# seervideodiffusion/SeerVideoLDM

Measured on AMD Instinct MI355X. Metric: UNet denoising steps/sec (12-frame 256^2 latent, 50-step DDIM), higher is better.
Workload: dtype bf16; 1 GPU; Sthv2 config: CFG batch 2 x 12 frames (2 cond + 10 predicted) x 32x32 latent, full-width SeerUNet 1.08G params, 50-step DDIM, scale 7.5; global_batch=1, parallelism=single, hip_graph=True

## Files before the change

include/seer_hip.h:

```cpp
#ifndef SEER_HIP_H
#define SEER_HIP_H

#include <stdint.h>

#ifdef __cplusplus
extern "C" {
#endif

#define SEER_OK 0
#define SEER_EINVAL (-22)
#define SEER_ENOSYS (-38)
#define SEER_ELAUNCH (-5)

#define SEER_DT_BF16 0
#define SEER_DT_F16 1

int seer_abi_version(void);
const char* seer_strerror(int code);
const char* seer_build_arch(void);

#define SEER_GEMM_PLAIN 0
#define SEER_GEMM_CONV3X3 1
#define SEER_EPI_GEGLU 1u
#define SEER_EPI_OUT_F32 2u
#define SEER_EPI_SILU 4u
#define SEER_EPI_TRANS_OUT 8u
#define SEER_EPI_ROTARY 16u
#define SEER_EPI_COLSCALE 32u

#define SEER_EPI_F16 64u
#define SEER_EPI_QUICKGELU 128u

typedef struct seer_gemm_desc {
    const void* A;
    const void* A2;
    const void* W;
    const float* bias;
    const void* residual;
    const float* rowvec;
    void* C;
    int32_t M, N, K, K1;
    int32_t lda, lda2, ldr, ldc;
    int32_t rows_per_batch, rowvec_ld;
    int32_t mode;
    uint32_t epilogue;
    int32_t Hin, Win, Cin, Hout, Wout, stride, upsample;
    int32_t batch;
    int64_t strideA, strideW, strideC;
    int32_t tile;
    int32_t splits;
    void* workspace;
    int64_t workspace_bytes;
    const float* rot_table;
    int32_t rot_tokens_per_batch, rot_pos_offset, rot_head_dim, rot_dim, rot_cols;
// ... 23 lines not shown
#define SEER_TILE_G64x64_3 8
#define SEER_TILE_G64x64_4 9
#define SEER_TILE_G64x64_5 10
#define SEER_TILE_G128x64_4 11
#define SEER_TILE_G128x160_2 12
#define SEER_TILE_G64x160_3 13
#define SEER_TILE_G256x128_2 14
#define SEER_TILE_G256x64_3 15
#define SEER_TILE_G96x160_2 16
#define SEER_TILE_G96x160_3 17
#define SEER_TILE_G96x128_2 18
#define SEER_TILE_G256x256_2 21
#define SEER_TILE_WS 19
#define SEER_TILE_T256x320 22
#define SEER_TILE_AUTO_TILED 20
#define SEER_TILE_AUTO_INVARIANT 23

int seer_gemm_bf16(const seer_gemm_desc* desc , void* stream);
int64_t seer_gemm_workspace_bytes(const seer_gemm_desc* desc );
int32_t seer_gemm_colsum_rows(const seer_gemm_desc* desc );
int32_t seer_gemm_colsum_fx_layout(const seer_gemm_desc* desc , int32_t rows_per_batch, int32_t* reps);
int32_t seer_gemm_rowstat_ok(const seer_gemm_desc* desc );
int32_t seer_gemm_lnfold_ok(const seer_gemm_desc* desc );
int64_t seer_gemm_sync_bytes(const seer_gemm_desc* desc );
#define SEER_GEMM_KERNEL_NONE 0
#define SEER_GEMM_KERNEL_TILE 1
#define SEER_GEMM_KERNEL_SPLITK 2
#define SEER_GEMM_KERNEL_WS 3
#define SEER_GEMM_KERNEL_T320 4
#define SEER_GEMM_REDUCE_NONE 0
#define SEER_GEMM_REDUCE_PLAIN 1
#define SEER_GEMM_REDUCE_COLSUM 2
#define SEER_GEMM_REDUCE_COLSUM_FX64 3
#define SEER_GEMM_REDUCE_COLSUM_FX32 4
int seer_gemm_plan(const seer_gemm_desc* desc , int32_t out[5]);

typedef struct seer_attn_desc {
    const void* Q; const void* K; const void* V; void* O;
    int64_t q_bs, k_bs, v_bs, o_bs;
    int32_t q_ss, k_ss, v_ss, o_ss;
    int32_t batch, heads, head_dim;
    int32_t Sq, Sk;
    int32_t causal;
    float scale;
    int32_t window_ws, F, H, W;
    int32_t Fq;
// ... 267 lines not shown
```

seervideoldm_amd/_lib.py:

```python
from __future__ import annotations

import ctypes as C
import os
from pathlib import Path

_PKG = Path(__file__).resolve().parent
_LIB_PATH = _PKG / "lib" / "libseer_hip.so"
_lib = None

ABI_VERSION = 27

SEER_GEMM_PLAIN = 0
SEER_GEMM_CONV3X3 = 1
SEER_EPI_GEGLU = 1
SEER_EPI_OUT_F32 = 2
SEER_EPI_SILU = 4
SEER_EPI_TRANS_OUT = 8
SEER_EPI_ROTARY = 16
SEER_EPI_COLSCALE = 32
SEER_EPI_F16 = 64
SEER_EPI_QUICKGELU = 128
SEER_ENOSYS = -38
SEER_INDEX_FROM_STEP = -1
SEER_DT_BF16, SEER_DT_F16 = 0, 1
SEER_ATTN_Q_PRESCALED = 1
SEER_ATTN_F16 = 2
SEER_TILE_AUTO, SEER_TILE_128x128, SEER_TILE_64x64, SEER_TILE_128x64 = 0, 1, 2, 3
SEER_TILE_WS = 19
SEER_TILE_AUTO_INVARIANT = 23
SEER_GEMM_KERNEL_NONE, SEER_GEMM_KERNEL_TILE, SEER_GEMM_KERNEL_SPLITK, SEER_GEMM_KERNEL_WS, SEER_GEMM_KERNEL_T320 = 0, 1, 2, 3, 4
SEER_GEMM_REDUCE_NONE, SEER_GEMM_REDUCE_PLAIN, SEER_GEMM_REDUCE_COLSUM, SEER_GEMM_REDUCE_COLSUM_FX64, SEER_GEMM_REDUCE_COLSUM_FX32 = 0, 1, 2, 3, 4


class SeerHipError(RuntimeError):
    pass


class GemmDesc(C.Structure):
    _fields_ = [
        ("A", C.c_void_p), ("A2", C.c_void_p), ("W", C.c_void_p), ("bias", C.c_void_p),
        ("residual", C.c_void_p), ("rowvec", C.c_void_p), ("C", C.c_void_p),
        ("M", C.c_int32), ("N", C.c_int32), ("K", C.c_int32), ("K1", C.c_int32),
        ("lda", C.c_int32), ("lda2", C.c_int32), ("ldr", C.c_int32), ("ldc", C.c_int32),
        ("rows_per_batch", C.c_int32), ("rowvec_ld", C.c_int32),
# ... 56 lines not shown
class AttnBwdDesc(C.Structure):
    _fields_ = [
        ("fwd", AttnDesc),
        ("dO", C.c_void_p), ("dQ", C.c_void_p), ("dK", C.c_void_p), ("dV", C.c_void_p),
        ("do_bs", C.c_int64), ("dq_bs", C.c_int64), ("dk_bs", C.c_int64), ("dv_bs", C.c_int64),
        ("do_ss", C.c_int32), ("dq_ss", C.c_int32), ("dk_ss", C.c_int32), ("dv_ss", C.c_int32),
        ("delta", C.c_void_p),
    ]


_vp, _i32, _i64, _f32, _f64 = C.c_void_p, C.c_int32, C.c_int64, C.c_float, C.c_double
_u32, _u64 = C.c_uint32, C.c_uint64

SIGNATURES = {
    "seer_abi_version": ([], C.c_int),
    "seer_strerror": ([C.c_int], C.c_char_p),
    "seer_build_arch": ([], C.c_char_p),
    "seer_gemm_bf16": ([C.POINTER(GemmDesc), _vp], C.c_int),
    "seer_gemm_workspace_bytes": ([C.POINTER(GemmDesc)], C.c_int64),
    "seer_gemm_colsum_rows": ([C.POINTER(GemmDesc)], C.c_int32),
    "seer_gemm_sync_bytes": ([C.POINTER(GemmDesc)], C.c_int64),
    "seer_gemm_rowstat_ok": ([C.POINTER(GemmDesc)], C.c_int32),
    "seer_gemm_lnfold_ok": ([C.POINTER(GemmDesc)], C.c_int32),
    "seer_gemm_plan": ([C.POINTER(GemmDesc), C.POINTER(C.c_int32)], C.c_int),
    "seer_attn_fwd": ([C.POINTER(AttnDesc), _vp], C.c_int),
    "seer_attn_causal64": ([_vp, _vp, _vp, _i32, _vp, _i32, _vp, _i32, _i32, _i32, _vp], C.c_int),
    "seer_embed_tokens": ([_vp, _i32, _i32, _vp, _i32, _vp, _i32, _i32, _vp, _i32, _vp], C.c_int),
    "seer_rotary_table": ([_vp, _i32, _i32, _vp, _vp], C.c_int),
    "seer_rotary_inplace": ([_vp, _i64, _i32, _i32, _i32, _i32, _i32, _i32, _i32, _i32, _vp, _vp], C.c_int),
    "seer_groupnorm_workspace_floats": ([_i32, _i32, _i64, _i32], C.c_int64),
    "seer_groupnorm_stats": ([_vp, _i32, _vp, _i32, _i32, _i64, _i32, _vp, _vp, _i32, _vp], C.c_int),
    "seer_groupnorm_stats_from_colsums": ([_vp, _i32, _i32, _i32, _vp, _i32, _i32, _i32, _i32, _i32, _vp, _vp], C.c_int),
    "seer_groupnorm_apply": ([_vp, _i32, _vp, _i32, _i32, _i64, _i32, _vp, _f64, _f32, _vp, _vp, _i32, _vp, _i32, _vp], C.c_int),
    "seer_groupnorm_apply_from_colsums": ([_vp, _i32, _vp, _i32, _vp, _i32, _i32, _vp, _i32, _i32, _i32, _i64, _i32, _f64, _f32, _vp, _vp, _i32,
                                           _vp, _i32, _vp], C.c_int),
    "seer_groupnorm_apply_fx": ([_vp, _i32, _vp, _i32, _vp, _i32, _vp, _i32, _i32, _i64, _i32, _f64, _f32, _vp, _vp, _i32, _vp, _vp, _i32, _vp],
                                 C.c_int),
    "seer_groupnorm_stats_fx": ([_vp, _i32, _i32, _i64, _vp, _i32, _vp], C.c_int),
    "seer_ff_fused_c320": ([_vp, _i32, _vp, _vp, _vp, _i32, _vp, _i32, _vp, _i32, _i64, _vp, _vp, C.c_float, _vp, _vp, _vp, _vp, _vp, _i64, _i32,
                            _vp, _i32, _vp], C.c_int),
    "seer_rowchain_c320": ([C.POINTER(RowChainDesc), _vp], C.c_int),
    "seer_rowchain_pack": ([_vp, _i32, _i32, _vp, _vp], C.c_int),
    "seer_ff_fused_pack_w1": ([_vp, _vp, _vp], C.c_int),
    "seer_ff_fused_pack_wcat": ([_vp, _vp, _vp], C.c_int),
    "seer_gemm_colsum_fx_layout": ([C.POINTER(GemmDesc), _i32, C.POINTER(C.c_int32)], C.c_int32),
    "seer_layernorm": ([_vp, _i64, _i32, _i32, _vp, _vp, _f32, _vp, _i32, _i32, _vp], C.c_int),
# ... 102 lines not shown
```

seervideoldm_amd/csrc/gemm.hip:

```cpp
#include "gemm_tiles.h"

namespace {

bool colsum_store_ok(const seer_gemm_desc& d) {
    return !(d.epilogue & (SEER_EPI_OUT_F32 | SEER_EPI_TRANS_OUT | SEER_EPI_GEGLU)) && d.ldc % 8 == 0 && d.N % 8 == 0 &&
           (reinterpret_cast<uintptr_t>(d.C) & 15) == 0 && (d.batch <= 1 || (d.strideC % 8) == 0);
}

int validate(seer_gemm_desc& d) {
    if (d.M <= 0 || d.N <= 0 || d.K <= 0) return SEER_EINVAL;
    if (d.K % BK) return SEER_EINVAL;
    if (!d.A || !d.W || !d.C) return SEER_EINVAL;
    const bool geglu = (d.epilogue & SEER_EPI_GEGLU) != 0;
    if (d.N % (geglu ? 32 : 4)) return SEER_EINVAL;
    if (d.mode == SEER_GEMM_CONV3X3) {
        if (d.Cin <= 0 || d.Cin % BK) return SEER_EINVAL;
        if (d.Hin <= 0 || d.Win <= 0 || d.Hout <= 0 || d.Wout <= 0) return SEER_EINVAL;
        if (d.upsample == 2) {
            if (d.K != 4 * d.Cin || d.stride != 1 || d.pad_after_only || d.Hout != 2 * d.Hin || d.Wout != 2 * d.Win) return SEER_EINVAL;
            if (d.M % (d.Hin * d.Win) || d.residual || d.rowvec) return SEER_EINVAL;
            if (d.epilogue & (SEER_EPI_OUT_F32 | SEER_EPI_TRANS_OUT | SEER_EPI_ROTARY | SEER_EPI_GEGLU)) return SEER_EINVAL;
            d.batch = 4;
            d.strideA = 0;
            d.strideW = (int64_t)d.N * d.K;
// ... 140 lines not shown
    if (d.mode != SEER_GEMM_PLAIN && d.mode != SEER_GEMM_CONV3X3) return 0;
    if (!seer_gemm_t320_eligible(d)) return 0;
    const bool geglu = (d.epilogue & SEER_EPI_GEGLU) != 0;
    const bool phases = d.mode == SEER_GEMM_CONV3X3 && d.upsample == 2;
    const bool can_split = !geglu && d.batch <= 1 && !phases && d.splits != 1;
    if (d.tile == SEER_TILE_T256x320) {
        if (!can_split) return 1;
        const int nk = d.K / BK;
        int s = d.splits > 1 ? d.splits : t320_best_split(d);
        if (s > nk / 4) s = nk / 4;
        if (s > 16) s = 16;
        if (s < 1) s = 1;
        const bool room = d.workspace && d.workspace_bytes >= seer_gemm_t320_workspace_bytes(d, s) && d.sync &&
                          d.sync_bytes >= seer_gemm_t320_sync_bytes(d, s);
        return (!assume_buffers && s > 1 && !room) ? 1 : s;
    }
    if (d.M % 256 || d.splits > 1) return 0;
    const double t = t320_model_us(d, 1);
    const double flops = 2.0 * d.M * d.N * (double)d.K * (phases ? 4 : d.batch > 1 ? d.batch : 1);
    const double rate = d.mode == SEER_GEMM_CONV3X3 ? 1.10e9 : geglu ? 0.78e9 : 0.85e9;
    return t < flops / rate ? 1 : 0;
}

struct tile_traits { int bm, bn; bool colsum_ok, ln_ok; };
tile_traits traits_of(int tile) {
    switch (tile) {
#define SEER_ROW(code, BM, BN, NS, WM, WN, MAY_SPLIT, UNIT) \
    case code: return {BM, BN, TileShape<BM, BN, NS, WM, WN>::colsum_ok, TileShape<BM, BN, NS, WM, WN>::ln_ok};
        SEER_GEMM_TILES(SEER_ROW)
#undef SEER_ROW
        default: return {};
    }
}

int launch_tiles(int tile, bool f16, const seer_gemm_desc& d, hipStream_t st) {
    switch (tile) {
#define SEER_ROW(code, BM, BN, NS, WM, WN, MAY_SPLIT, UNIT)                                                    \
    case code:                                                                                                 \
        static_assert(UNIT >= 0 && UNIT < SEER_GEMM_TILE_UNITS && (!MAY_SPLIT || (WM == 2 && WN == 2)), #code); \
        return seer_gemm_tiles_launch<UNIT>(tile, f16, d, st);
        SEER_GEMM_TILES(SEER_ROW)
#undef SEER_ROW
        default: return SEER_EINVAL;
    }
}

bool ln_resolve(const seer_gemm_desc& d, const tile_traits& tile) {
    const bool geglu = (d.epilogue & SEER_EPI_GEGLU) != 0;
    if (d.mode != SEER_GEMM_PLAIN || d.batch > 1 || (d.epilogue & (SEER_EPI_OUT_F32 | SEER_EPI_TRANS_OUT | SEER_EPI_SILU | SEER_EPI_QUICKGELU)))
        return false;
    if (d.ldc % 8 || d.N % (geglu ? 16 : 8) || (reinterpret_cast<uintptr_t>(d.C) & 15)) return false;
    if (d.rowstat && (geglu || d.colsum || d.colsum_fx)) return false;
    if (d.ln_rowstat && (d.A2 || !d.ln_wsum || (reinterpret_cast<uintptr_t>(d.ln_wsum) & 15))) return false;
    return tile.ln_ok;
}

split_choice invariant_split(const seer_gemm_desc& d) {
    const int nk = d.K / BK;
    const bool can_split = d.batch == 1 && !(d.epilogue & (SEER_EPI_GEGLU | SEER_EPI_TRANS_OUT | SEER_EPI_ROTARY)) && d.splits != 1 &&
                           !d.rowstat && !d.ln_rowstat;
    if (!can_split) return {1, SEER_TILE_AUTO};
    if (d.splits > 1) return {d.splits < nk ? d.splits : nk, SEER_TILE_G64x64_3};
    const bool conv = d.mode == SEER_GEMM_CONV3X3;
    if (conv && d.N % 160 == 0 && d.N >= 1024 && nk >= 88) return {4, SEER_TILE_G96x160_2};
    if (conv && d.N % 160 == 0 && d.N >= 512 && d.N < 1024 && nk >= 80) return {2, SEER_TILE_G96x160_2};
    if (!conv && d.N % 128 == 0 && d.N >= 1024 && nk >= 88) return {4, SEER_TILE_G128x128_2};
    return {1, SEER_TILE_AUTO};
// ... 53 lines not shown
    if (s320) {
        take(SEER_GEMM_KERNEL_T320, SEER_TILE_T256x320, s320);
    } else if (slices && !rows_ln) {
        take(SEER_GEMM_KERNEL_SPLITK, sc.tile, sc.splits);
        p.reduce = !d.colsum_fx ? (d.colsum ? SEER_GEMM_REDUCE_COLSUM : SEER_GEMM_REDUCE_PLAIN)
                 : splitk_fx_rows(d.M, inv) == 64 ? SEER_GEMM_REDUCE_COLSUM_FX64 : SEER_GEMM_REDUCE_COLSUM_FX32;
    } else {
        const bool ws = !sums && !rows_ln && seer_gemm_ws_eligible(d) &&
                        (requested == SEER_TILE_WS || (requested == SEER_TILE_AUTO && seer_gemm_ws_profitable(d)));
        take(ws ? SEER_GEMM_KERNEL_WS : SEER_GEMM_KERNEL_TILE, inv ? invariant_tile(d) : resolve_tile(d), 1);
        tile = traits_of(p.tile);
    }
    p.ln_ok = rows_ln && ln_resolve(d, tile);
    const bool split = p.kernel == SEER_GEMM_KERNEL_SPLITK;
    const int rows = !sums_stored ? 0 : s320 ? (d.M % 256 ? 0 : s320 > 1 ? 16 : 64)
                   : (p.kernel == SEER_GEMM_KERNEL_TILE && tile.colsum_ok) ? tile.bm : 0;
    p.colsum_rows = slices && sums_stored ? splitk_cs_rows(d.M, inv) : rows;
    p.colsum_fx_rows = slices && sums_stored ? splitk_fx_rows(d.M, inv) : rows;
    const bool fx_bad = d.colsum_fx && (d.colsum || d.colsum_fx_reps < 1 || d.colsum_fx_rows <= 0 || d.M % d.colsum_fx_rows ||
                                        !p.colsum_fx_rows || d.colsum_fx_rows % p.colsum_fx_rows);
    const bool sums_bad = sums && (split ? (d.epilogue & (SEER_EPI_OUT_F32 | SEER_EPI_TRANS_OUT | SEER_EPI_GEGLU)) != 0 : !rows);
    const bool tile_bad = !s320 && !split && (!tile.bm || (geglu && (d.mode == SEER_GEMM_CONV3X3 || (tile.bn / 32) % 2)));
    if (fx_bad || sums_bad || tile_bad || (rows_ln && !p.ln_ok)) p.status = SEER_EINVAL;
    if (inv) {
        if (split && !assume_buffers && !room) p.status = SEER_EINVAL;
        d.tile = SEER_TILE_AUTO_INVARIANT;
    }
    return p;
}

}

extern "C" int seer_gemm_plan(const seer_gemm_desc* desc, int32_t out[5]) {
    if (!desc || !out) return SEER_EINVAL;
    const gemm_plan p = plan_gemm(*desc, false);
    const bool ok = p.status == SEER_OK;
    out[0] = p.status; out[1] = ok ? p.kernel : 0; out[2] = ok ? p.tile : 0; out[3] = ok ? p.splits : 0; out[4] = ok ? p.reduce : 0;
    return SEER_OK;
}

extern "C" int64_t seer_gemm_workspace_bytes(const seer_gemm_desc* desc) {
    if (!desc) return SEER_EINVAL;
    const gemm_plan p = plan_gemm(*desc, true);
    if (p.kernel == SEER_GEMM_KERNEL_NONE) return p.status;
    const int s = p.tile_splits;
    const int64_t w320 = p.kernel == SEER_GEMM_KERNEL_T320 ? seer_gemm_t320_workspace_bytes(p.d, p.splits) : 0;
// ... 19 lines not shown
    if (!desc || rows_per_batch <= 0 || desc->M % rows_per_batch) return 0;
    seer_gemm_desc d = *desc;
    if (!d.colsum && !d.colsum_fx) d.colsum_fx = reinterpret_cast<int64_t*>(16);
    const int rows = plan_gemm(d, false).colsum_fx_rows;
    if (rows <= 0 || rows_per_batch % rows) return 0;
    const int adds = rows_per_batch / rows;
    if (reps) *reps = adds <= 24 ? 1 : adds <= 48 ? 2 : adds <= 96 ? 4 : 8;
    return rows;
}

extern "C" int32_t seer_gemm_rowstat_ok(const seer_gemm_desc* desc) {
    if (!desc) return 0;
    seer_gemm_desc d = *desc;
    if (!d.rowstat) d.rowstat = reinterpret_cast<int64_t*>(16);
    return plan_gemm(d, false).ln_ok ? 1 : 0;
}

extern "C" int32_t seer_gemm_lnfold_ok(const seer_gemm_desc* desc) {
    if (!desc || !desc->ln_rowstat) return 0;
    seer_gemm_desc d = *desc;
    d.ln_rowstat = nullptr;
    if (d.tile == SEER_TILE_AUTO && plan_gemm(d, false).kernel == SEER_GEMM_KERNEL_WS) return 0;
    return plan_gemm(*desc, false).ln_ok ? 1 : 0;
}

extern "C" int seer_gemm_bf16(const seer_gemm_desc* desc, void* stream) {
    if (!desc) return SEER_EINVAL;
    gemm_plan p = plan_gemm(*desc, false);
    if (p.status != SEER_OK) return p.status;
    p.d.splits = p.splits;
    hipStream_t st = reinterpret_cast<hipStream_t>(stream);
    const bool f16 = (p.d.epilogue & SEER_EPI_F16) != 0;
    switch (p.kernel) {
        case SEER_GEMM_KERNEL_T320: return seer_gemm_t320_launch(p.d, p.splits, st);
        case SEER_GEMM_KERNEL_SPLITK:
            if (const int rc = launch_tiles(p.tile, f16, p.d, st); rc != SEER_OK) return rc;
            return seer_gemm_reduce_launch(p.d, p.reduce, st);
        case SEER_GEMM_KERNEL_WS:
            if (const int rc = seer_gemm_ws_launch(p.d, st); rc != SEER_ENOSYS) return rc;
            [[fallthrough]];
        default:
            return launch_tiles(p.tile, f16, p.d, st);
    }
}
```

seervideoldm_amd/csrc/gemm_tile_kernel.h:

```cpp
#pragma once
#include "gemm_tiles.h"
#include <mutex>
#include <type_traits>

#ifdef SEER_GEMM_STAMPS
__device__ long long seer_pp8_stamps[64 * 8 * 16];
extern "C" long long* seer_lab_pp8_stamps() {
    long long* p = nullptr;
    (void)hipGetSymbolAddress(reinterpret_cast<void**>(&p), HIP_SYMBOL(seer_pp8_stamps));
    return p;
}
__device__ long long seer_block_span[8192 * 2];
extern "C" long long* seer_lab_block_span() {
    long long* p = nullptr;
    (void)hipGetSymbolAddress(reinterpret_cast<void**>(&p), HIP_SYMBOL(seer_block_span));
    return p;
}
#define PSPAN(which)                                                                                                   \
    do {                                                                                                               \
        if (threadIdx.x == 0 && blockIdx.z == 0 && blockIdx.x < 8192) seer_block_span[blockIdx.x * 2 + (which)] = wall_clock64(); \
    } while (0)
#define PSTAMP()                                                                                                       \
    do {                                                                                                               \
        if (blockIdx.x < 64 && blockIdx.z == 0 && (threadIdx.x & 63) == 0 && nst_ < 16)                                \
// ... 28 lines not shown

    extern __shared__ __attribute__((aligned(16))) unsigned char smem[];
    constexpr int STAGE = TS::STAGE;
    bf16* const smem_b = reinterpret_cast<bf16*>(smem);

    [[maybe_unused]] int nst_ = 0;
    const int tid = threadIdx.x;
    const int lane = tid & 63;
    const int wave = __builtin_amdgcn_readfirstlane(tid >> 6);
    const int wm = wave / WN, wn = wave % WN;
    PSTAMP();
    PSPAN(0);

    const int tiles_m = (p.M + BM - 1) / BM;
    const int tiles_n = (p.N + BN - 1) / BN;
    const int nwg = tiles_m * tiles_n;
    int wg;
    {
        const int L = blockIdx.x;
        const int xcd = L & 7;
        const int q = nwg >> 3, r = nwg & 7;
        wg = (xcd < r ? xcd * (q + 1) : r * (q + 1) + (xcd - r) * q) + (L >> 3);
    }
#ifndef SEER_GEMM_GM
#define SEER_GEMM_GM 4
#endif
    constexpr int GM = SEER_GEMM_GM;
    const int group = wg / (GM * tiles_n);
    const int first_m = group * GM;
    const int gsz = min(tiles_m - first_m, GM);
    const int tm = first_m + (wg % (GM * tiles_n)) % gsz;
    const int tn = (wg % (GM * tiles_n)) / gsz;
    const int m0 = tm * BM, n0 = tn * BN;

    const int z = SPLIT ? 0 : blockIdx.z;
    const bf16* __restrict__ A = reinterpret_cast<const bf16*>(p.A) + (int64_t)z * p.strideA;
    const bf16* __restrict__ A2 = reinterpret_cast<const bf16*>(p.A2);
    const bf16* __restrict__ W = reinterpret_cast<const bf16*>(p.W) + (int64_t)z * p.strideW;

    const int c8 = (tid & 7) * 8;
    const int srow = tid >> 3;
    int64_t a_off[A_CH];
    int64_t a_off2[A_CH];
    int a_oy[A_CH], a_ox[A_CH];
    auto a_tile_row = [&](int c) { return PP8 ? (wave >> 2) * 128 + (c >> 1) * 64 + 16 * (wave & 3) + 8 * (c & 1) + (lane >> 3) : srow + RPP * c; };
    auto b_tile_row = [&](int c) {
        const int hn = 16 * wave + 8 * (c & 1) + (lane >> 3);
        return PP8 ? (hn >> 5) * 64 + (c >> 1) * 32 + (hn & 31) : srow + RPP * c;
    };
// ... 428 lines not shown
            if constexpr (P32) {
#pragma unroll
                for (int ks = 0; ks < 2; ++ks)
#pragma unroll
                    for (int h = 0; h < 2; ++h)
#pragma unroll
                        for (int i = 0; i < TM / 2; ++i)
#pragma unroll
                            for (int j = 0; j < TN / 2; ++j)
                                acc32[i][j] = __builtin_amdgcn_mfma_f32_32x32x16_bf16(wf[ks][2 * j + h], af[ks][2 * i + h], acc32[i][j], 0, 0, 0);
                return;
            }
#endif
#pragma unroll
            for (int ks = 0; ks < 2; ++ks)
#pragma unroll
                for (int i = 0; i < TM; ++i)
#pragma unroll
                    for (int j = 0; j < TN; ++j)
                        acc[i][j] = mma16<F16>(wf[ks][j], af[ks][i], acc[i][j]);
        };
        {
        PSTAMP();
#pragma unroll
        for (int s_ = 0; s_ < NS; ++s_)
            if (kt0 + s_ < nk) issue_tile(kt0 + s_, s_);
#if SEER_GEMM_PROBE & 2
        read_frags(0);
#endif
        int stage = 0;
        for (int kt = kt0; kt < nk; ++kt) {
            const int pending = min(NS - 1, nk - 1 - kt);
            if (NS >= 4 && pending >= 3) asm volatile("s_waitcnt vmcnt(%0)" ::"n"(3 * LPT) : "memory");
            else if (NS >= 3 && pending == 2) asm volatile("s_waitcnt vmcnt(%0)" ::"n"(2 * LPT) : "memory");
            else if (pending == 1) asm volatile("s_waitcnt vmcnt(%0)" ::"n"(LPT) : "memory");
            else asm volatile("s_waitcnt vmcnt(0)" ::: "memory");
            asm volatile("s_barrier" ::: "memory");
#ifdef SEER_GEMM_STAMPS
            if (kt == kt0) PSTAMP();
#endif
#if !(SEER_GEMM_PROBE & 2)
            read_frags(stage);
#endif
            asm volatile("s_waitcnt lgkmcnt(0)" ::: "memory");
            asm volatile("s_barrier" ::: "memory");
#if !(SEER_GEMM_PROBE & 1)
            if (kt + NS < nk) issue_tile(kt + NS, stage);
#endif
#if !(SEER_GEMM_PROBE & 4)
// ... 418 lines not shown
                        int64_t* o = fx_slot(p, m0 / BM, m0) + n0o + tid;
                        fx_add(o, sm);
                        fx_add(o + p.N, sq);
                    } else {
                        const int tiles_m = (p.M + BM - 1) / BM;
                        float* o = p.colsum + (((int64_t)blockIdx.z * tiles_m + m0 / BM) * p.N + n0o + tid) * 2;
                        *reinterpret_cast<f32x2*>(o) = f32x2{sm, sq};
                    }
                }
            }
        }
    }
    PSTAMP();
    PSPAN(1);
}

template <int BM, int BN, int NS, int WM, int WN, bool F16>
std::once_flag g_tile_lds_once;

template <int BM, int BN, int NS, int WM = 2, int WN = 2, bool F16 = false>
int launch_tile(const seer_gemm_desc& d, hipStream_t st) {
    const int tiles_m = (d.M + BM - 1) / BM, tiles_n = (d.N + BN - 1) / BN;
    dim3 grid(tiles_m * tiles_n, 1, d.batch > 1 ? d.batch : 1);
    const size_t lds = TileShape<BM, BN, NS, WM, WN>::RING_BYTES;
    constexpr bool GEGLU_OK = TileShape<BM, BN, NS, WM, WN>::GEGLU_OK;
    if (lds > 64 * 1024) {
        std::call_once(g_tile_lds_once<BM, BN, NS, WM, WN, F16>, [lds] {
            (void)hipFuncSetAttribute(reinterpret_cast<const void*>(&seer_gemm_kernel<BM, BN, true, false, false, NS, WM, WN, F16>),
                                      hipFuncAttributeMaxDynamicSharedMemorySize, (int)lds);
            if constexpr (GEGLU_OK)
                (void)hipFuncSetAttribute(reinterpret_cast<const void*>(&seer_gemm_kernel<BM, BN, false, true, false, NS, WM, WN, F16>),
                                          hipFuncAttributeMaxDynamicSharedMemorySize, (int)lds);
            (void)hipFuncSetAttribute(reinterpret_cast<const void*>(&seer_gemm_kernel<BM, BN, false, false, false, NS, WM, WN, F16>),
                                      hipFuncAttributeMaxDynamicSharedMemorySize, (int)lds);
        });
    }
    const bool conv = d.mode == SEER_GEMM_CONV3X3;
    const bool geglu = (d.epilogue & SEER_EPI_GEGLU) != 0;
    if (conv) {
        hipLaunchKernelGGL((seer_gemm_kernel<BM, BN, true, false, false, NS, WM, WN, F16>), grid, dim3(64 * WM * WN), lds, st, d);
    } else if (geglu) {
        if constexpr (GEGLU_OK)
            hipLaunchKernelGGL((seer_gemm_kernel<BM, BN, false, true, false, NS, WM, WN, F16>), grid, dim3(64 * WM * WN), lds, st, d);
        else
            return SEER_EINVAL;
    } else {
        hipLaunchKernelGGL((seer_gemm_kernel<BM, BN, false, false, false, NS, WM, WN, F16>), grid, dim3(64 * WM * WN), lds, st, d);
    }
    SEER_LAUNCH_CHECK();
    return SEER_OK;
}

template <int BM, int BN, int NS, bool F16 = false>
int launch_split_tile(const seer_gemm_desc& d, hipStream_t st) {
    const int tiles_m = (d.M + BM - 1) / BM, tiles_n = (d.N + BN - 1) / BN;
    dim3 grid(tiles_m * tiles_n, 1, d.splits);
    const size_t lds = TileShape<BM, BN, NS>::RING_BYTES;
    if (d.mode == SEER_GEMM_CONV3X3)
        hipLaunchKernelGGL((seer_gemm_kernel<BM, BN, true, false, true, NS, 2, 2, F16>), grid, dim3(256), lds, st, d);
    else
        hipLaunchKernelGGL((seer_gemm_kernel<BM, BN, false, false, true, NS, 2, 2, F16>), grid, dim3(256), lds, st, d);
    SEER_LAUNCH_CHECK();
    return SEER_OK;
}

}
```

seervideoldm_amd/csrc/gemm_tiles.h:

```cpp
#pragma once
#include "seer_common.h"

#define SEER_GEMM_TILES(X)                            \
    X(SEER_TILE_128x128, 128, 128, 0, 2, 2, false, 4)    \
    X(SEER_TILE_128x64, 128, 64, 0, 2, 2, false, 2)      \
    X(SEER_TILE_64x64, 64, 64, 0, 2, 2, true, 3)         \
    X(SEER_TILE_G128x128_2, 128, 128, 2, 2, 2, true, 1)  \
    X(SEER_TILE_G128x128_3, 128, 128, 3, 2, 2, false, 2) \
    X(SEER_TILE_G128x64_3, 128, 64, 3, 2, 2, false, 1)   \
    X(SEER_TILE_G64x64_3, 64, 64, 3, 2, 2, true, 5)      \
    X(SEER_TILE_G64x64_4, 64, 64, 4, 2, 2, false, 0)     \
    X(SEER_TILE_G64x64_5, 64, 64, 5, 2, 2, false, 4)     \
    X(SEER_TILE_G128x64_4, 128, 64, 4, 2, 2, false, 2)   \
    X(SEER_TILE_G128x160_2, 128, 160, 2, 2, 2, false, 5) \
    X(SEER_TILE_G64x160_3, 64, 160, 3, 2, 2, false, 1)   \
    X(SEER_TILE_G256x128_2, 256, 128, 2, 4, 2, false, 3) \
    X(SEER_TILE_G256x64_3, 256, 64, 3, 4, 2, false, 0)   \
    X(SEER_TILE_G256x256_2, 256, 256, 2, 2, 4, false, 0) \
    X(SEER_TILE_G96x160_2, 96, 160, 2, 2, 2, true, 5)    \
    X(SEER_TILE_G96x160_3, 96, 160, 3, 2, 2, false, 3)   \
    X(SEER_TILE_G96x128_2, 96, 128, 2, 2, 2, false, 4)
constexpr int SEER_GEMM_TILE_UNITS = 6;

template <int U>
int seer_gemm_tiles_launch(int tile, bool f16, const seer_gemm_desc& d, hipStream_t st);
int seer_gemm_reduce_launch(const seer_gemm_desc& d, int reduce, hipStream_t st);

bool seer_gemm_ws_eligible(const seer_gemm_desc& d);
bool seer_gemm_ws_profitable(const seer_gemm_desc& d);
int seer_gemm_ws_launch(const seer_gemm_desc& d, hipStream_t st);
bool seer_gemm_t320_eligible(const seer_gemm_desc& d);
int64_t seer_gemm_t320_workspace_bytes(const seer_gemm_desc& d, int splits);
int64_t seer_gemm_t320_sync_bytes(const seer_gemm_desc& d, int splits);
int seer_gemm_t320_launch(const seer_gemm_desc& d, int splits, hipStream_t st);

__host__ __device__ inline int splitk_cs_rows(int M, bool inv) { return (inv || M >= 2048) ? 16 : 4; }
__host__ inline int splitk_fx_rows(int M, bool inv) { return (!inv && M >= 1024) ? 64 : 32; }

namespace {

constexpr int BK = 64;

template <int BM_, int BN_, int NS_, int WM_ = 2, int WN_ = 2>
struct TileShape {
    static constexpr int BM = BM_, BN = BN_, NS = NS_, WM = WM_, WN = WN_;
    static constexpr int NT = 64 * WM * WN;
    static constexpr int STAGE = (BM + BN) * BK;
    static constexpr int RING_BYTES = (NS == 0 ? 2 : NS) * STAGE * (int)sizeof(bf16);
    static constexpr bool PP8 = WM == 2 && WN == 4 && BM == 256 && BN == 256;
    static constexpr bool GEGLU_OK = ((BN / 32) % 2) == 0;
    static constexpr int bno(bool geglu) { return geglu ? BN / 2 : BN; }
    static constexpr bool cswz(bool geglu) { return BM * (bno(geglu) * 2 + 16) > 2 * STAGE * (int)sizeof(bf16); }
    static constexpr int cpitch(bool geglu) { return bno(geglu) * 2 + (cswz(geglu) ? 0 : 16); }
    static constexpr int lnrow_off(bool geglu) { return BM * cpitch(geglu) + 4096; }
    static constexpr bool colsum_ok = !PP8 && BN <= NT && BM * cpitch(false) + (NT / (BN / 2)) * BN * 8 <= RING_BYTES;
    static constexpr bool ln_ok = !PP8 && BM <= NT && lnrow_off(false) + BM * 8 <= RING_BYTES;
};

}
```

seervideoldm_amd/ops.py:

```python
from __future__ import annotations

import ctypes as C
from typing import Optional

import torch

from . import _lib
from ._lib import SEER_INDEX_FROM_STEP, AttnDesc, GemmDesc, check

bf16 = torch.bfloat16


def _stream() -> int:
    return torch.cuda.current_stream().cuda_stream


def _p(t: Optional[torch.Tensor]) -> Optional[int]:
    if t is None:
        return None
    if not t.is_cuda:
        raise _lib.SeerHipError("seervideoldm_amd kernels need tensors on a ROCm device (no CPU fallback)")
    return t.data_ptr()


# ... 72 lines not shown
        self.used = 0

    def take_rows(self, rows: int) -> Optional[torch.Tensor]:
        n = rows * 2
        if self.used + n > self.buf.numel():
            return None
        t = self.buf[self.used:self.used + n].view(rows, 2)
        self.used += n
        self.high = max(self.high, self.used)
        return t

    def take(self, reps: int, batch: int, C_: int) -> Optional[torch.Tensor]:
        n = reps * batch * C_ * 2
        if self.used + n > self.buf.numel():
            return None
        t = self.buf[self.used:self.used + n].view(reps, batch, 2, C_)
        self.used += n
        self.high = max(self.high, self.used)
        return t


def gemm(a: torch.Tensor, w: torch.Tensor, *, bias=None, residual=None, rowvec=None, rows_per_batch=0,
         a2: Optional[torch.Tensor] = None, geglu=False, silu=False, out_f32=False, out: Optional[torch.Tensor] = None,
         tile=0, splits=0, rotary=None, col_scale=None, colsum_batch=0, rowstat=False, ln=None, quick_gelu=False) -> Optional[torch.Tensor]:
    dt = _req16(a, "a"); _req16(w, "w", a)
    assert a.dim() == 2 and w.dim() == 2 and a.stride(1) == 1 and w.is_contiguous()
    M, K1 = a.shape
    N, K = w.shape
    d = GemmDesc()
    d.A, d.W = _p(a), _p(w)
    d.lda = a.stride(0)
    if a2 is not None:
        _req16(a2, "a2", a)
        assert a2.shape[0] == M and a2.stride(1) == 1 and K1 + a2.shape[1] == K
        d.A2, d.lda2 = _p(a2), a2.stride(0)
    else:
        assert K1 == K, f"K mismatch {K1} vs {K}"
    d.M, d.N, d.K, d.K1 = M, N, K, K1
    n_out = N // 2 if geglu else N
    if out is None:
        out = torch.empty((M, n_out), device=a.device, dtype=torch.float32 if out_f32 else a.dtype)
    assert out.shape == (M, n_out) and out.stride(1) == 1
    d.C, d.ldc = _p(out), out.stride(0)
    if bias is not None:
        _req(bias, torch.float32, "bias"); d.bias = _p(bias)
    if residual is not None:
        _req16(residual, "residual", a)
        assert residual.shape == (M, n_out) and residual.stride(1) == 1
        d.residual, d.ldr = _p(residual), residual.stride(0)
    if rowvec is not None:
        _req(rowvec, torch.float32, "rowvec")
        assert rowvec.dim() == 2 and rowvec.stride(1) == 1
        d.rowvec, d.rowvec_ld, d.rows_per_batch = _p(rowvec), rowvec.stride(0), rows_per_batch
    d.mode = _lib.SEER_GEMM_PLAIN
    d.epilogue = (_lib.SEER_EPI_GEGLU if geglu else 0) | (_lib.SEER_EPI_SILU if silu else 0) | \
                 (_lib.SEER_EPI_QUICKGELU if quick_gelu else 0) | \
                 (_lib.SEER_EPI_OUT_F32 if (out.dtype == torch.float32) else 0) | (_lib.SEER_EPI_F16 if dt else 0)
    assert out.dtype in (torch.float32, a.dtype)
    if rotary is not None:
        table, tpb, pos_off, hd, rd, cols = rotary
        _req(table, torch.float32, "rotary table")
        assert table.shape[0] >= tpb + pos_off and table.shape[1] * 2 == rd
        d.epilogue |= _lib.SEER_EPI_ROTARY
        d.rot_table, d.rot_tokens_per_batch, d.rot_pos_offset = _p(table), tpb, pos_off
        d.rot_head_dim, d.rot_dim, d.rot_cols = hd, rd, cols
    if col_scale is not None:
        d.epilogue |= _lib.SEER_EPI_COLSCALE
        d.col_scale, d.col_scale_cols = float(col_scale[0]), int(col_scale[1])
    d.batch = 1
    d.tile = tile
    d.splits = splits
    lib = _lib.load()
    if ln is not None:
        rs, wsum, eps = ln
        _req(wsum, torch.float32, "ln wsum")
        assert rs.buf.shape[0] == M and wsum.shape[0] == N and a2 is None
        d.ln_rowstat, d.ln_wsum, d.ln_eps = _p(rs.buf), _p(wsum), float(eps)
        if not lib.seer_gemm_lnfold_ok(C.byref(d)):
            return None
    rstats = None
    if rowstat and lib.seer_gemm_rowstat_ok(C.byref(d)):
        buf = rowstat.take_rows(M) if isinstance(rowstat, FxArena) else None
        if buf is None:
            buf = torch.zeros((M, 2), device=a.device, dtype=torch.int64)
        rstats = RowStats(buf)
        d.rowstat = _p(buf)
    cs = _launch_gemm(d, a.device, "seer_gemm_bf16", colsum_batch)
    out.colsums = cs
    out.rowstats = rstats
    return out


_SYNC_BYTES = 1 << 16
_sync_buffers: dict = {}


def _sync_buffer(device) -> torch.Tensor:
    key = (device.type, device.index if device.index is not None else torch.cuda.current_device())
    buf = _sync_buffers.get(key)
    if buf is None:
        assert not torch.cuda.is_current_stream_capturing(), "the split-K counter buffer must exist before a graph capture"
        buf = torch.zeros((_SYNC_BYTES,), device=device, dtype=torch.uint8)
        _sync_buffers[key] = buf
    return buf


def _launch_gemm(d: GemmDesc, device, what: str, colsum_batch: int = 0) -> Optional[ColSums]:
    lib = _lib.load()
    nbytes = lib.seer_gemm_workspace_bytes(C.byref(d))
    if nbytes < 0:
        check(int(nbytes), what)
    if nbytes > 0:
        ws = torch.empty((nbytes // 4,), device=device, dtype=torch.float32)
# ... 7 lines not shown
    arena = None
    if isinstance(colsum_batch, tuple):
        colsum_batch, arena = colsum_batch
    if colsum_batch > 0 and d.M % colsum_batch == 0:
        fx = None
        if arena is not None:
            reps = C.c_int32(1)
            if lib.seer_gemm_colsum_fx_layout(C.byref(d), d.M // colsum_batch, C.byref(reps)) > 0:
                fx = arena.take(reps.value, colsum_batch, int(d.N))
        if fx is not None:
            d.colsum_fx, d.colsum_fx_rows, d.colsum_fx_reps = fx.data_ptr(), d.M // colsum_batch, fx.shape[0]
            cs = ColSumsFx(fx, int(d.N))
        rows = 0 if fx is not None else lib.seer_gemm_colsum_rows(C.byref(d))
        if rows > 0 and (d.M // colsum_batch) % rows == 0:
            phases, tiles = max(int(d.batch), 1), d.M // rows
            buf = torch.empty((phases, tiles, d.N, 2), device=device, dtype=torch.float32)
            d.colsum = buf.data_ptr()
            cs = ColSums(buf, int(d.N), phases, tiles)
    check(lib.seer_gemm_bf16(C.byref(d), _stream()), what)
    return cs


def gemm_batched(a: torch.Tensor, w: torch.Tensor, *, trans_out=False, out: Optional[torch.Tensor] = None,
                 bias: Optional[torch.Tensor] = None, out_f32=False, tile=0, col_scale=None) -> torch.Tensor:
    dt = _req16(a, "a"); _req16(w, "w", a)
    assert a.dim() == 3 and a.is_contiguous() and w.is_contiguous()
    Bt, M, K = a.shape
    N = w.shape[-2]
    d = GemmDesc()
    d.A, d.W = _p(a), _p(w)
    d.lda = K
    d.M, d.N, d.K, d.K1 = M, N, K, K
    if out is None:
        out = torch.empty((Bt, N, M) if trans_out else (Bt, M, N), device=a.device,
                          dtype=torch.float32 if out_f32 else a.dtype)
    d.C = _p(out)
    if bias is not None:
        _req(bias, torch.float32, "bias"); d.bias = _p(bias)
    d.ldc = M if trans_out else N
    d.batch = Bt
    d.strideA = M * K
    d.strideW = N * K if w.dim() == 3 else 0
    d.strideC = M * N
    d.epilogue = (_lib.SEER_EPI_TRANS_OUT if trans_out else 0) | (_lib.SEER_EPI_OUT_F32 if out.dtype == torch.float32 else 0) | \
                 (_lib.SEER_EPI_F16 if dt else 0)
    if col_scale is not None:
        d.epilogue |= _lib.SEER_EPI_COLSCALE
        d.col_scale, d.col_scale_cols = float(col_scale[0]), int(col_scale[1])
    d.tile = tile
    check(_lib.load().seer_gemm_bf16(C.byref(d), _stream()), "seer_gemm_bf16(batched)")
    return out


def conv3x3(x: torch.Tensor, w: torch.Tensor, n_img: int, Hin: int, Win: int, *, stride=1, upsample=False,
            bias=None, residual=None, rowvec=None, rows_per_batch=0, out: Optional[torch.Tensor] = None,
            tile=0, splits=0, pad_after_only=False, colsum_batch=0) -> torch.Tensor:
    dt = _req16(x, "x"); _req16(w, "w", x)
    assert x.is_contiguous() and w.is_contiguous()
    Cin = x.shape[1]
    Cout, K = w.shape
    assert K == 9 * Cin and x.shape[0] == n_img * Hin * Win
    Hs, Ws = (2 * Hin, 2 * Win) if upsample else (Hin, Win)
    pad = 1 if pad_after_only else 2
    Ho, Wo = (Hs + pad - 3) // stride + 1, (Ws + pad - 3) // stride + 1
    M = n_img * Ho * Wo
    d = GemmDesc()
    d.A, d.W = _p(x), _p(w)
    d.M, d.N, d.K, d.K1 = M, Cout, K, K
    if out is None:
        out = torch.empty((M, Cout), device=x.device, dtype=x.dtype)
    d.C, d.ldc = _p(out), out.stride(0)
    if bias is not None:
        _req(bias, torch.float32, "bias"); d.bias = _p(bias)
    if residual is not None:
        _req16(residual, "residual", x)
        assert residual.shape == (M, Cout) and residual.stride(1) == 1
        d.residual, d.ldr = _p(residual), residual.stride(0)
    if rowvec is not None:
        _req(rowvec, torch.float32, "rowvec")
        d.rowvec, d.rowvec_ld, d.rows_per_batch = _p(rowvec), rowvec.stride(0), rows_per_batch
    d.mode = _lib.SEER_GEMM_CONV3X3
    d.epilogue = _lib.SEER_EPI_F16 if dt else 0
    d.Hin, d.Win, d.Cin, d.Hout, d.Wout, d.stride, d.upsample = Hin, Win, Cin, Ho, Wo, stride, int(upsample)
    d.pad_after_only = int(pad_after_only)
    d.batch = 1
    d.tile = tile
    d.splits = splits
    cs = _launch_gemm(d, x.device, "seer_gemm_bf16(conv3x3)", colsum_batch)
    out.colsums = cs
    return out


def conv_up2x(x: torch.Tensor, w4: torch.Tensor, n_img: int, Hin: int, Win: int, *, bias=None,
              out: Optional[torch.Tensor] = None, tile=0, colsum_batch=0) -> torch.Tensor:
    dt = _req16(x, "x"); _req16(w4, "w4", x)
    assert x.is_contiguous() and w4.is_contiguous()
    Cin = x.shape[1]
    four, Cout, K = w4.shape
    assert four == 4 and K == 4 * Cin and x.shape[0] == n_img * Hin * Win
    d = GemmDesc()
    d.A, d.W = _p(x), _p(w4)
    d.M, d.N, d.K, d.K1 = n_img * Hin * Win, Cout, K, K
    if out is None:
        out = torch.empty((n_img * 4 * Hin * Win, Cout), device=x.device, dtype=x.dtype)
    d.C, d.ldc = _p(out), out.stride(0)
    if bias is not None:
        _req(bias, torch.float32, "bias"); d.bias = _p(bias)
    d.mode = _lib.SEER_GEMM_CONV3X3
    d.epilogue = _lib.SEER_EPI_F16 if dt else 0
    d.Hin, d.Win, d.Cin, d.Hout, d.Wout, d.stride, d.upsample = Hin, Win, Cin, 2 * Hin, 2 * Win, 1, 2
    d.batch = 4
    d.tile = tile
    d.splits = 1
    cs = _launch_gemm(d, x.device, "seer_gemm_bf16(conv_up2x)", colsum_batch)
    out.colsums = cs
    return out


def attention(q: torch.Tensor, k: torch.Tensor, v: torch.Tensor, out: torch.Tensor, *, batch: int, heads: int,
              head_dim: int, Sq: int, Sk: int, causal=False, scale: Optional[float] = None,
              window=None, Fq: Optional[int] = None, causal_offset: int = 0,
              seq_stride_rows: int = 1, batch_stride_rows: Optional[int] = None,
              lse: Optional[torch.Tensor] = None, q_prescaled: bool = False, variant: int = 0,
              q_head_major: bool = False, kv_head_major: bool = False, _desc_only: bool = False) -> torch.Tensor:
    dt = _req16(q, "q")
    for t, n in ((k, "k"), (v, "v"), (out, "out")):
        _req16(t, n, q)
    for t in (q, k, v, out):
        assert t.dim() == 2 and t.stride(1) == 1
    d = AttnDesc()
    d.Q, d.K, d.V, d.O = _p(q), _p(k), _p(v), _p(out)
    d.q_ss, d.k_ss, d.v_ss, d.o_ss = q.stride(0), k.stride(0), v.stride(0), out.stride(0)
# ... 992 lines not shown
```

Before: 102.4 steps/s.

## Prefetch weight panel into cache with cooperative touch loads across M-tiles

```diff
diff --git a/include/seer_hip.h b/include/seer_hip.h
--- a/include/seer_hip.h
+++ b/include/seer_hip.h
@@ -30,6 +30,8 @@
 
 #define SEER_EPI_F16 64u
 #define SEER_EPI_QUICKGELU 128u
+#define SEER_EPI_W_TOUCH 256u
+#define SEER_EPI_W_TOUCH_OFF 512u
 
 typedef struct seer_gemm_desc {
     const void* A;
@@ -99,6 +101,7 @@
 int32_t seer_gemm_colsum_fx_layout(const seer_gemm_desc* desc , int32_t rows_per_batch, int32_t* reps);
 int32_t seer_gemm_rowstat_ok(const seer_gemm_desc* desc );
 int32_t seer_gemm_lnfold_ok(const seer_gemm_desc* desc );
+int32_t seer_gemm_w_touch(const seer_gemm_desc* desc );
 int64_t seer_gemm_sync_bytes(const seer_gemm_desc* desc );
 #define SEER_GEMM_KERNEL_NONE 0
 #define SEER_GEMM_KERNEL_TILE 1
diff --git a/seervideoldm_amd/_lib.py b/seervideoldm_amd/_lib.py
--- a/seervideoldm_amd/_lib.py
+++ b/seervideoldm_amd/_lib.py
@@ -20,6 +20,8 @@
 SEER_EPI_COLSCALE = 32
 SEER_EPI_F16 = 64
 SEER_EPI_QUICKGELU = 128
+SEER_EPI_W_TOUCH = 256
+SEER_EPI_W_TOUCH_OFF = 512
 SEER_ENOSYS = -38
 SEER_INDEX_FROM_STEP = -1
 SEER_DT_BF16, SEER_DT_F16 = 0, 1
@@ -122,6 +124,7 @@
     "seer_gemm_sync_bytes": ([C.POINTER(GemmDesc)], C.c_int64),
     "seer_gemm_rowstat_ok": ([C.POINTER(GemmDesc)], C.c_int32),
     "seer_gemm_lnfold_ok": ([C.POINTER(GemmDesc)], C.c_int32),
+    "seer_gemm_w_touch": ([C.POINTER(GemmDesc)], C.c_int32),
     "seer_gemm_plan": ([C.POINTER(GemmDesc), C.POINTER(C.c_int32)], C.c_int),
     "seer_attn_fwd": ([C.POINTER(AttnDesc), _vp], C.c_int),
     "seer_attn_causal64": ([_vp, _vp, _vp, _i32, _vp, _i32, _vp, _i32, _i32, _i32, _vp], C.c_int),
diff --git a/seervideoldm_amd/csrc/gemm.hip b/seervideoldm_amd/csrc/gemm.hip
--- a/seervideoldm_amd/csrc/gemm.hip
+++ b/seervideoldm_amd/csrc/gemm.hip
@@ -186,11 +186,15 @@
     return t < flops / rate ? 1 : 0;
 }
 
-struct tile_traits { int bm, bn; bool colsum_ok, ln_ok; };
+constexpr bool W_TOUCH_AUTO = true;
+constexpr int W_TOUCH_MIN_BEYOND = 2;
+constexpr int W_TOUCH_MIN_SHARERS = 6;
+
+struct tile_traits { int bm, bn; bool colsum_ok, ln_ok; int ns; bool touch_ok; };
 tile_traits traits_of(int tile) {
     switch (tile) {
 #define SEER_ROW(code, BM, BN, NS, WM, WN, MAY_SPLIT, UNIT) \
-    case code: return {BM, BN, TileShape<BM, BN, NS, WM, WN>::colsum_ok, TileShape<BM, BN, NS, WM, WN>::ln_ok};
+    case code: return {BM, BN, TileShape<BM, BN, NS, WM, WN>::colsum_ok, TileShape<BM, BN, NS, WM, WN>::ln_ok, NS, TileShape<BM, BN, NS, WM, WN>::touch_ok};
         SEER_GEMM_TILES(SEER_ROW)
 #undef SEER_ROW
         default: return {};
@@ -207,6 +211,19 @@
 #undef SEER_ROW
         default: return SEER_EINVAL;
     }
+}
+
+bool w_touch_on(const seer_gemm_desc& d, int kernel, int tile, int splits) {
+    if (d.epilogue & SEER_EPI_W_TOUCH_OFF) return false;
+    if (kernel != SEER_GEMM_KERNEL_TILE && kernel != SEER_GEMM_KERNEL_SPLITK) return false;
+    const tile_traits t = traits_of(tile);
+    if (!t.touch_ok) return false;
+    const int nk = d.K / BK, s = splits > 1 ? splits : 1;
+    const int beyond = (nk + s - 1) / s - t.ns;
+    if (beyond <= 0) return false;
+    if ((int64_t)t.bn * d.K * 2 >= ((int64_t)1 << 31)) return false;
+    if (d.epilogue & SEER_EPI_W_TOUCH) return true;
+    return W_TOUCH_AUTO && beyond >= W_TOUCH_MIN_BEYOND && (d.M + t.bm - 1) / t.bm >= W_TOUCH_MIN_SHARERS && !(d.epilogue & SEER_EPI_GEGLU);
 }
 
 bool ln_resolve(const seer_gemm_desc& d, const tile_traits& tile) {
@@ -306,6 +323,8 @@
     const bool sums_bad = sums && (split ? (d.epilogue & (SEER_EPI_OUT_F32 | SEER_EPI_TRANS_OUT | SEER_EPI_GEGLU)) != 0 : !rows);
     const bool tile_bad = !s320 && !split && (!tile.bm || (geglu && (d.mode == SEER_GEMM_CONV3X3 || (tile.bn / 32) % 2)));
     if (fx_bad || sums_bad || tile_bad || (rows_ln && !p.ln_ok)) p.status = SEER_EINVAL;
+    const bool touch = w_touch_on(d, p.kernel, p.tile, p.splits);
+    d.epilogue = (d.epilogue & ~(SEER_EPI_W_TOUCH | SEER_EPI_W_TOUCH_OFF)) | (touch ? SEER_EPI_W_TOUCH : 0u);
     if (inv) {
         if (split && !assume_buffers && !room) p.status = SEER_EINVAL;
         d.tile = SEER_TILE_AUTO_INVARIANT;
@@ -371,6 +390,12 @@
     d.ln_rowstat = nullptr;
     if (d.tile == SEER_TILE_AUTO && plan_gemm(d, false).kernel == SEER_GEMM_KERNEL_WS) return 0;
     return plan_gemm(*desc, false).ln_ok ? 1 : 0;
+}
+
+extern "C" int32_t seer_gemm_w_touch(const seer_gemm_desc* desc) {
+    if (!desc) return 0;
+    const gemm_plan p = plan_gemm(*desc, false);
+    return p.status == SEER_OK && (p.d.epilogue & SEER_EPI_W_TOUCH) ? 1 : 0;
 }
 
 extern "C" int seer_gemm_bf16(const seer_gemm_desc* desc, void* stream) {
diff --git a/seervideoldm_amd/csrc/gemm_tile_kernel.h b/seervideoldm_amd/csrc/gemm_tile_kernel.h
--- a/seervideoldm_amd/csrc/gemm_tile_kernel.h
+++ b/seervideoldm_amd/csrc/gemm_tile_kernel.h
@@ -74,9 +74,6 @@
         const int q = nwg >> 3, r = nwg & 7;
         wg = (xcd < r ? xcd * (q + 1) : r * (q + 1) + (xcd - r) * q) + (L >> 3);
     }
-#ifndef SEER_GEMM_GM
-#define SEER_GEMM_GM 4
-#endif
     constexpr int GM = SEER_GEMM_GM;
     const int group = wg / (GM * tiles_n);
     const int first_m = group * GM;
@@ -551,9 +548,26 @@
         };
         {
         PSTAMP();
+        auto touch_panel = [&]() {
+        if constexpr (TS::touch_ok) {
+                if (p.epilogue & SEER_EPI_W_TOUCH) {
+                    const w_touch_geom tg = w_touch_geometry(p.N, BN, NS, tn, kt0, nk, SEER_W_TOUCH_CAP);
+                    int t_R, t_me;
+                    w_touch_sharers(tiles_m, tm, GM, &t_R, &t_me);
+                    unsigned char* const t_lds = smem + TS::RING_BYTES + wave * 256;
+                    for (int c = t_me + t_R * wave; c < tg.chunks; c += t_R * (NT / 64)) {
+                        const unsigned off = w_touch_offset(tg, p.K, c, lane);
+                        if (off != SEER_W_TOUCH_NONE)
+                            __builtin_amdgcn_raw_ptr_buffer_load_lds(r_w, (__attribute__((address_space(3))) void*)t_lds, 4, (int)off, 0, 0, 0);
+                    }
+                }
+            }
+        };
+        if (!SEER_W_TOUCH_AFTER) touch_panel();
 #pragma unroll
         for (int s_ = 0; s_ < NS; ++s_)
             if (kt0 + s_ < nk) issue_tile(kt0 + s_, s_);
+        if (SEER_W_TOUCH_AFTER) touch_panel();
 #if SEER_GEMM_PROBE & 2
         read_frags(0);
 #endif
@@ -1018,10 +1032,12 @@
 int launch_tile(const seer_gemm_desc& d, hipStream_t st) {
     const int tiles_m = (d.M + BM - 1) / BM, tiles_n = (d.N + BN - 1) / BN;
     dim3 grid(tiles_m * tiles_n, 1, d.batch > 1 ? d.batch : 1);
-    const size_t lds = TileShape<BM, BN, NS, WM, WN>::RING_BYTES;
-    constexpr bool GEGLU_OK = TileShape<BM, BN, NS, WM, WN>::GEGLU_OK;
+    using TS = TileShape<BM, BN, NS, WM, WN>;
+    const size_t lds = TS::RING_BYTES + (TS::touch_ok && (d.epilogue & SEER_EPI_W_TOUCH) ? TS::TOUCH_BYTES : 0);
+    constexpr bool GEGLU_OK = TS::GEGLU_OK;
     if (lds > 64 * 1024) {
-        std::call_once(g_tile_lds_once<BM, BN, NS, WM, WN, F16>, [lds] {
+        std::call_once(g_tile_lds_once<BM, BN, NS, WM, WN, F16>, [] {
+            constexpr int lds = TS::RING_BYTES + (TS::touch_ok ? TS::TOUCH_BYTES : 0);
             (void)hipFuncSetAttribute(reinterpret_cast<const void*>(&seer_gemm_kernel<BM, BN, true, false, false, NS, WM, WN, F16>),
                                       hipFuncAttributeMaxDynamicSharedMemorySize, (int)lds);
             if constexpr (GEGLU_OK)
@@ -1047,11 +1063,24 @@
     return SEER_OK;
 }
 
+template <int BM, int BN, int NS, bool F16>
+std::once_flag g_split_lds_once;
+
 template <int BM, int BN, int NS, bool F16 = false>
 int launch_split_tile(const seer_gemm_desc& d, hipStream_t st) {
     const int tiles_m = (d.M + BM - 1) / BM, tiles_n = (d.N + BN - 1) / BN;
     dim3 grid(tiles_m * tiles_n, 1, d.splits);
-    const size_t lds = TileShape<BM, BN, NS>::RING_BYTES;
+    using TS = TileShape<BM, BN, NS>;
+    const size_t lds = TS::RING_BYTES + (TS::touch_ok && (d.epilogue & SEER_EPI_W_TOUCH) ? TS::TOUCH_BYTES : 0);
+    if (lds > 64 * 1024) {
+        std::call_once(g_split_lds_once<BM, BN, NS, F16>, [] {
+            constexpr int most = TS::RING_BYTES + TS::TOUCH_BYTES;
+            (void)hipFuncSetAttribute(reinterpret_cast<const void*>(&seer_gemm_kernel<BM, BN, true, false, true, NS, 2, 2, F16>),
+                                      hipFuncAttributeMaxDynamicSharedMemorySize, most);
+            (void)hipFuncSetAttribute(reinterpret_cast<const void*>(&seer_gemm_kernel<BM, BN, false, false, true, NS, 2, 2, F16>),
+                                      hipFuncAttributeMaxDynamicSharedMemorySize, most);
+        });
+    }
     if (d.mode == SEER_GEMM_CONV3X3)
         hipLaunchKernelGGL((seer_gemm_kernel<BM, BN, true, false, true, NS, 2, 2, F16>), grid, dim3(256), lds, st, d);
     else
diff --git a/seervideoldm_amd/csrc/gemm_tiles.h b/seervideoldm_amd/csrc/gemm_tiles.h
--- a/seervideoldm_amd/csrc/gemm_tiles.h
+++ b/seervideoldm_amd/csrc/gemm_tiles.h
@@ -1,5 +1,12 @@
 #pragma once
+#ifndef SEER_GEMM_TILES_PLAIN_HOST
 #include "seer_common.h"
+#endif
+#if defined(__HIPCC__)
+#define SEER_HD __host__ __device__
+#else
+#define SEER_HD
+#endif
 
 #define SEER_GEMM_TILES(X)                            \
     X(SEER_TILE_128x128, 128, 128, 0, 2, 2, false, 4)    \
@@ -22,6 +29,51 @@
     X(SEER_TILE_G96x128_2, 96, 128, 2, 2, 2, false, 4)
 constexpr int SEER_GEMM_TILE_UNITS = 6;
 
+#ifndef SEER_W_TOUCH_CAP
+#define SEER_W_TOUCH_CAP 16
+#endif
+#ifndef SEER_W_TOUCH_SCOPE_GROUP
+#define SEER_W_TOUCH_SCOPE_GROUP 0
+#endif
+#ifndef SEER_W_TOUCH_AFTER
+#define SEER_W_TOUCH_AFTER 1
+#endif
+#ifndef SEER_GEMM_GM
+#define SEER_GEMM_GM 4
+#endif
+constexpr unsigned SEER_W_TOUCH_NONE = 0x80000000u;
+struct w_touch_geom { int first, tiles, rows, chunks; };
+SEER_HD inline void w_touch_slice(int nk_all, int slice, int splits, int* kt0, int* kt1) {
+    *kt0 = splits > 1 ? (int)((long long)nk_all * slice / splits) : 0;
+    *kt1 = splits > 1 ? (int)((long long)nk_all * (slice + 1) / splits) : nk_all;
+}
+SEER_HD inline w_touch_geom w_touch_geometry(int N, int bn, int ns, int tn, int kt0, int kt1, int cap) {
+    w_touch_geom g;
+    g.first = kt0 + ns;
+    const int end = kt1 < g.first + cap ? kt1 : g.first + cap;
+    g.tiles = end > g.first ? end - g.first : 0;
+    g.rows = N - tn * bn < bn ? N - tn * bn : bn;
+    g.chunks = g.tiles > 0 && g.rows > 0 ? (g.rows * g.tiles + 63) / 64 : 0;
+    return g;
+}
+SEER_HD inline unsigned w_touch_offset(const w_touch_geom& g, int K, int chunk, int lane) {
+    const int L = chunk * 64 + lane;
+    if (L >= g.rows * g.tiles) return SEER_W_TOUCH_NONE;
+    const int r = L / g.tiles, t = L - r * g.tiles;
+    return (unsigned)r * (unsigned)K * 2u + (unsigned)(g.first + t) * 128u;
+}
+SEER_HD inline void w_touch_sharers(int tiles_m, int tm, int gm, int* R, int* me) {
+    if (SEER_W_TOUCH_SCOPE_GROUP) {
+        const int first_m = tm / gm * gm;
+        *R = tiles_m - first_m < gm ? tiles_m - first_m : gm;
+        *me = tm - first_m;
+    } else {
+        *R = tiles_m;
+        *me = tm;
+    }
+}
+
+#ifndef SEER_GEMM_TILES_PLAIN_HOST
 template <int U>
 int seer_gemm_tiles_launch(int tile, bool f16, const seer_gemm_desc& d, hipStream_t st);
 int seer_gemm_reduce_launch(const seer_gemm_desc& d, int reduce, hipStream_t st);
@@ -55,6 +107,9 @@
     static constexpr int lnrow_off(bool geglu) { return BM * cpitch(geglu) + 4096; }
     static constexpr bool colsum_ok = !PP8 && BN <= NT && BM * cpitch(false) + (NT / (BN / 2)) * BN * 8 <= RING_BYTES;
     static constexpr bool ln_ok = !PP8 && BM <= NT && lnrow_off(false) + BM * 8 <= RING_BYTES;
+    static constexpr int TOUCH_BYTES = (NT / 64) * 256;
+    static constexpr bool touch_ok = NS >= 2 && !PP8 && (160 * 1024) / RING_BYTES == (160 * 1024) / (RING_BYTES + TOUCH_BYTES);
 };
 
 }
+#endif
diff --git a/seervideoldm_amd/ops.py b/seervideoldm_amd/ops.py
--- a/seervideoldm_amd/ops.py
+++ b/seervideoldm_amd/ops.py
@@ -118,7 +118,8 @@
 
 def gemm(a: torch.Tensor, w: torch.Tensor, *, bias=None, residual=None, rowvec=None, rows_per_batch=0,
          a2: Optional[torch.Tensor] = None, geglu=False, silu=False, out_f32=False, out: Optional[torch.Tensor] = None,
-         tile=0, splits=0, rotary=None, col_scale=None, colsum_batch=0, rowstat=False, ln=None, quick_gelu=False) -> Optional[torch.Tensor]:
+         tile=0, splits=0, rotary=None, col_scale=None, colsum_batch=0, rowstat=False, ln=None, quick_gelu=False,
+         w_touch: Optional[bool] = None) -> Optional[torch.Tensor]:
     dt = _req16(a, "a"); _req16(w, "w", a)
     assert a.dim() == 2 and w.dim() == 2 and a.stride(1) == 1 and w.is_contiguous()
     M, K1 = a.shape
@@ -163,6 +164,7 @@
     if col_scale is not None:
         d.epilogue |= _lib.SEER_EPI_COLSCALE
         d.col_scale, d.col_scale_cols = float(col_scale[0]), int(col_scale[1])
+    d.epilogue |= _w_touch_bits(w_touch)
     d.batch = 1
     d.tile = tile
     d.splits = splits
@@ -185,6 +187,10 @@
     out.colsums = cs
     out.rowstats = rstats
     return out
+
+
+def _w_touch_bits(w_touch: Optional[bool]) -> int:
+    return 0 if w_touch is None else _lib.SEER_EPI_W_TOUCH if w_touch else _lib.SEER_EPI_W_TOUCH_OFF
 
 
 _SYNC_BYTES = 1 << 16
@@ -238,7 +244,8 @@
 
 
 def gemm_batched(a: torch.Tensor, w: torch.Tensor, *, trans_out=False, out: Optional[torch.Tensor] = None,
-                 bias: Optional[torch.Tensor] = None, out_f32=False, tile=0, col_scale=None) -> torch.Tensor:
+                 bias: Optional[torch.Tensor] = None, out_f32=False, tile=0, col_scale=None,
+                 w_touch: Optional[bool] = None) -> torch.Tensor:
     dt = _req16(a, "a"); _req16(w, "w", a)
     assert a.dim() == 3 and a.is_contiguous() and w.is_contiguous()
     Bt, M, K = a.shape
@@ -259,7 +266,7 @@
     d.strideW = N * K if w.dim() == 3 else 0
     d.strideC = M * N
     d.epilogue = (_lib.SEER_EPI_TRANS_OUT if trans_out else 0) | (_lib.SEER_EPI_OUT_F32 if out.dtype == torch.float32 else 0) | \
-                 (_lib.SEER_EPI_F16 if dt else 0)
+                 (_lib.SEER_EPI_F16 if dt else 0) | _w_touch_bits(w_touch)
     if col_scale is not None:
         d.epilogue |= _lib.SEER_EPI_COLSCALE
         d.col_scale, d.col_scale_cols = float(col_scale[0]), int(col_scale[1])
@@ -270,7 +277,7 @@
 
 def conv3x3(x: torch.Tensor, w: torch.Tensor, n_img: int, Hin: int, Win: int, *, stride=1, upsample=False,
             bias=None, residual=None, rowvec=None, rows_per_batch=0, out: Optional[torch.Tensor] = None,
-            tile=0, splits=0, pad_after_only=False, colsum_batch=0) -> torch.Tensor:
+            tile=0, splits=0, pad_after_only=False, colsum_batch=0, w_touch: Optional[bool] = None) -> torch.Tensor:
     dt = _req16(x, "x"); _req16(w, "w", x)
     assert x.is_contiguous() and w.is_contiguous()
     Cin = x.shape[1]
@@ -296,7 +303,7 @@
         _req(rowvec, torch.float32, "rowvec")
         d.rowvec, d.rowvec_ld, d.rows_per_batch = _p(rowvec), rowvec.stride(0), rows_per_batch
     d.mode = _lib.SEER_GEMM_CONV3X3
-    d.epilogue = _lib.SEER_EPI_F16 if dt else 0
+    d.epilogue = (_lib.SEER_EPI_F16 if dt else 0) | _w_touch_bits(w_touch)
     d.Hin, d.Win, d.Cin, d.Hout, d.Wout, d.stride, d.upsample = Hin, Win, Cin, Ho, Wo, stride, int(upsample)
     d.pad_after_only = int(pad_after_only)
     d.batch = 1
@@ -308,7 +315,7 @@
 
 
 def conv_up2x(x: torch.Tensor, w4: torch.Tensor, n_img: int, Hin: int, Win: int, *, bias=None,
-              out: Optional[torch.Tensor] = None, tile=0, colsum_batch=0) -> torch.Tensor:
+              out: Optional[torch.Tensor] = None, tile=0, colsum_batch=0, w_touch: Optional[bool] = None) -> torch.Tensor:
     dt = _req16(x, "x"); _req16(w4, "w4", x)
     assert x.is_contiguous() and w4.is_contiguous()
     Cin = x.shape[1]
@@ -323,7 +330,7 @@
     if bias is not None:
         _req(bias, torch.float32, "bias"); d.bias = _p(bias)
     d.mode = _lib.SEER_GEMM_CONV3X3
-    d.epilogue = _lib.SEER_EPI_F16 if dt else 0
+    d.epilogue = (_lib.SEER_EPI_F16 if dt else 0) | _w_touch_bits(w_touch)
     d.Hin, d.Win, d.Cin, d.Hout, d.Wout, d.stride, d.upsample = Hin, Win, Cin, 2 * Hin, 2 * Win, 1, 2
     d.batch = 4
     d.tile = tile
```

Measured after the change: 102.9 steps/s, median of 6. No clear change (+0.4%).
